# kristofbc/physical-interaction-video-prediction

Measured on AMD Instinct MI355X. Metric: predicted frames/sec (64x64x3, 10-step rollout), higher is better.
Workload: dtype f32; 1 GPU; CDNA rollout forward (Model.__call__, feed-self), batch 32/GPU, 10-frame 64x64x3 sequences, action-conditioned, num_masks=10, random-init weights; global_batch=32, parallelism=replicas x1

## Files before the change

physical-interaction-video-prediction_amd/csrc/igemm_small.hip:

```cpp
#include <stdlib.h>
#include <type_traits>

#include "pivp_kernels.h"

namespace pivp {

namespace {
constexpr int SP = 36;
constexpr int TILE = 32 * SP;
}

template <int NTB, bool IN_LN = false, bool FUSE3 = false>
__global__ __launch_bounds__(256) void igemm_small_kernel(const IgemmDesc d) {
    static_assert(!FUSE3 || NTB == 2, "the fused 1x1 needs all 64 channels of a pixel in one block");
    const int bx = blockIdx.x, by = blockIdx.y, gdy = gridDim.y;
    PIVP_SET_MAIN_PRIO();
    constexpr int BN = 32 * NTB;
    constexpr int RP = BN + 4;
    constexpr int A_OFF = 0, B_OFF = 2 * TILE;
    constexpr int STAGE_FLOATS = 2 * TILE + 2 * NTB * TILE, RED_FLOATS = 4 * 32 * RP;
    __shared__ __attribute__((aligned(16))) float lds[STAGE_FLOATS > RED_FLOATS ? STAGE_FLOATS : RED_FLOATS];
    const int tid = threadIdx.x, lane = tid & 63;
    const int wave = __builtin_amdgcn_readfirstlane(tid >> 6);
    const int half = lane >> 5, l31 = lane & 31;
    const int n_nblk = d.n_mblk;
    const int mblk = pivp_fdiv(bx, d.fd_mb_mul, d.fd_mb_sh), nblk = bx - mblk * n_nblk;
    const int m0 = mblk * 32;
    const int phase = by, py = phase >> 1, px = phase & 1;
    const bool deconv = d.deconv != 0;
    const int nty = deconv ? 1 + py : d.ksize, ntx = deconv ? 1 + px : d.ksize;
    const int ncc = (d.c0 + d.c1) >> 5;
    const int nchunks = nty * ntx * ncc;
    const int HWg = d.Hg * d.Wg;

    constexpr unsigned OOB = 0xC0000000u;
    const int cvec = tid & 7, prow = tid >> 3;
    const __amdgpu_buffer_rsrc_t rs0 = __builtin_amdgcn_make_buffer_rsrc(const_cast<float*>(d.x0), 0, d.bytes0, 0x00020000);
    const __amdgpu_buffer_rsrc_t rs1 = __builtin_amdgcn_make_buffer_rsrc(const_cast<float*>(d.c1 ? d.x1 : d.x0), 0, d.c1 ? d.bytes1 : d.bytes0, 0x00020000);
    const __amdgpu_buffer_rsrc_t rsw = __builtin_amdgcn_make_buffer_rsrc(const_cast<float*>(d.w), 0, d.bytesw, 0x00020000);
    int a_off0 = 0, a_off1 = 0, a_iy0 = -(1 << 20), a_ix0 = 0, a_pix0 = 0;
    auto anchor = [&]() {
        const int m = m0 + prow;
        if (m < d.M) {
            const int b = pivp_fdiv(m, d.fd_hw_mul, d.fd_hw_sh), rem = m - b * HWg;
            const int ay = pivp_fdiv(rem, d.fd_w_mul, d.fd_w_sh), ax = rem - ay * d.Wg;
            a_iy0 = ay * d.in_step; a_ix0 = ax * d.in_step;
            const int pix = b * d.Hin * d.Win + a_iy0 * d.Win + a_ix0;
            a_pix0 = pix;
            a_off0 = (pix * d.ld0 + cvec * 4) * 4;
            a_off1 = (pix * d.ld1 + cvec * 4) * 4;
        }
    };
    int b_goff[NTB];
#pragma unroll
    for (int t = 0; t < NTB; ++t) b_goff[t] = ((nblk * BN + t * 32 + prow) * 32 + cvec * 4) * 4;
    const int lds_w = prow * SP + cvec * 4;

    constexpr bool in_ln = IN_LN;
    __shared__ float in_stat[2];
    const __amdgpu_buffer_rsrc_t rsg = __builtin_amdgcn_make_buffer_rsrc(const_cast<float*>(in_ln ? d.in_g : d.x0), 0, in_ln ? d.Hin * d.Win * d.c0 * 4 : 0, 0x00020000);
    const __amdgpu_buffer_rsrc_t rsb = __builtin_amdgcn_make_buffer_rsrc(const_cast<float*>(in_ln ? d.in_b : d.x0), 0, in_ln ? d.Hin * d.Win * d.c0 * 4 : 0, 0x00020000);
    if (IN_LN && tid < 64) {
        float mean, rstd;
        ln_merge_partials(d.in_part, pivp_fdiv(m0, d.fd_hw_mul, d.fd_hw_sh), d.in_np, d.in_eps, mean, rstd);
        if (tid == 0) {
            in_stat[0] = mean; in_stat[1] = rstd;
            const int bs = pivp_fdiv(m0, d.fd_hw_mul, d.fd_hw_sh);
            if (d.in_stat_out && nblk == 0 && m0 == bs * HWg) { d.in_stat_out[bs * 2] = mean; d.in_stat_out[bs * 2 + 1] = rstd; }
        }
    }
    int l_cc = 0, l_ty = 0, l_tx = 0;
    constexpr int NS = 4;
    f32x4 ras[NS], rbs[NS][NTB];
    f32x4 rgs[NS], rbe[NS];
    int roo[NS];
    auto load_next = [&](auto SET, auto PART) {
        constexpr int part = decltype(PART)::value;
        f32x4& ra = ras[decltype(SET)::value];
        f32x4 (&rb)[NTB] = rbs[decltype(SET)::value];
        int dy, dx, wi;
        if (deconv) {
            const int ky = py ? 2 * l_ty : 1, kx = px ? 2 * l_tx : 1;
            dy = (py + 1 - ky) >> 1; dx = (px + 1 - kx) >> 1; wi = ky * 3 + kx;
        } else {
            dy = l_ty - d.pad; dx = l_tx - d.pad; wi = l_ty * d.ksize + l_tx;
        }
        const int ch = l_cc << 5;
        const bool first = ch < d.c0;
        const int ld = first ? d.ld0 : d.ld1;
        const int delta = ((dy * d.Win + dx) * ld + (first ? ch : ch - d.c0)) * 4;
        const int wbase = (wi * (d.wcin >> 5) + l_cc) * (d.wN ? d.wN : d.N) * 128;
        if constexpr (part != 1) {
            const int iy = a_iy0 + dy, ix = a_ix0 + dx;
            const bool ok = (unsigned)iy < (unsigned)d.Hin && (unsigned)ix < (unsigned)d.Win;
            const unsigned off = ok ? (unsigned)((first ? a_off0 : a_off1) + delta) : OOB;
            ra = __builtin_bit_cast(f32x4, first ? __builtin_amdgcn_raw_buffer_load_b128(rs0, off, 0, 0)
                                                 : __builtin_amdgcn_raw_buffer_load_b128(rs1, off, 0, 0));
            if constexpr (IN_LN) {
                const bool own = d.in_out && nblk == 0 && ok && l_ty >= 1 && l_tx >= 1 && l_ty < nty;
                roo[decltype(SET)::value] = own ? (a_pix0 + dy * d.Win + dx) * d.in_out_ld + ch + cvec * 4 : -1;
                const unsigned goff = ok ? (unsigned)(((iy * d.Win + ix) * d.c0 + ch + cvec * 4) * 4) : OOB;
                rgs[decltype(SET)::value] = __builtin_bit_cast(f32x4, __builtin_amdgcn_raw_buffer_load_b128(rsg, goff, 0, 0));
                rbe[decltype(SET)::value] = __builtin_bit_cast(f32x4, __builtin_amdgcn_raw_buffer_load_b128(rsb, goff, 0, 0));
            }
        }
        if constexpr (part != 2) {
#pragma unroll
            for (int t = 0; t < NTB; ++t) rb[t] = __builtin_bit_cast(f32x4, __builtin_amdgcn_raw_buffer_load_b128(rsw, b_goff[t], wbase, 0));
        }
        if constexpr (part != 1) { if (++l_cc == ncc) { l_cc = 0; if (++l_tx == ntx) { l_tx = 0; ++l_ty; } } }
    };
    auto store_regs = [&](auto SET, int buf) {
        f32x4 ra = ras[decltype(SET)::value];
        const f32x4 (&rb)[NTB] = rbs[decltype(SET)::value];
        if constexpr (IN_LN) {
            const float mean = in_stat[0], rstd = in_stat[1];
            const f32x4 g = rgs[decltype(SET)::value], be = rbe[decltype(SET)::value];
#pragma unroll
            for (int e = 0; e < 4; ++e) ra[e] = (ra[e] - mean) * rstd * g[e] + be[e];
            if (d.in_out && roo[decltype(SET)::value] >= 0) *reinterpret_cast<f32x4*>(d.in_out + roo[decltype(SET)::value]) = ra;
        }
        *reinterpret_cast<f32x4*>(lds + A_OFF + buf * TILE + lds_w) = ra;
#pragma unroll
        for (int t = 0; t < NTB; ++t) *reinterpret_cast<f32x4*>(lds + B_OFF + (buf * NTB + t) * TILE + lds_w) = rb[t];
    };

    if (nchunks > 0) load_next(std::integral_constant<int, 0>{}, std::integral_constant<int, 1>{});
    __builtin_amdgcn_sched_barrier(0);
    anchor();
    float f3w[FUSE3 ? 16 : 1], f3c = 0.f;
    if constexpr (FUSE3) {
        const int col = 16 * wave + (lane & 15), kg = lane >> 4, bs = pivp_fdiv(m0, d.fd_hw_mul, d.fd_hw_sh);
#pragma unroll
        for (int s4 = 0; s4 < 16; ++s4) f3w[s4] = d.f3_w[(4 * s4 + kg) * 64 + col];
        f3c = d.f3_b[col];
        if (d.f3_use_state) {
#pragma unroll
            for (int j = 0; j < 10; ++j) f3c = fmaf(j < 5 ? d.f3_action[bs * 5 + j] : d.f3_state[bs * 5 + j - 5], d.f3_w[(64 + j) * 64 + col], f3c);
        }
    }
    f32x16 acc[NTB];
#pragma unroll
    for (int t = 0; t < NTB; ++t)
#pragma unroll
        for (int r = 0; r < 16; ++r) acc[t][r] = 0.f;
    const int frag = l31 * SP + 8 * wave + 4 * half;

    if (nchunks > 0) {
        using S0 = std::integral_constant<int, 0>; using S1 = std::integral_constant<int, 1>;
        using P0 = std::integral_constant<int, 0>; using P2 = std::integral_constant<int, 2>;
        auto mma = [&](int buf) {
            const f32x4 fa = *reinterpret_cast<const f32x4*>(lds + A_OFF + buf * TILE + frag);
            f32x4 fb[NTB];
#pragma unroll
            for (int t = 0; t < NTB; ++t) fb[t] = *reinterpret_cast<const f32x4*>(lds + B_OFF + (buf * NTB + t) * TILE + frag);
#pragma unroll
            for (int s2 = 0; s2 < 4; ++s2)
#pragma unroll
                for (int t = 0; t < NTB; ++t) acc[t] = __builtin_amdgcn_mfma_f32_32x32x2f32(fa[s2], fb[t][s2], acc[t], 0, 0, 0);
        };
        using S2 = std::integral_constant<int, 2>; using S3 = std::integral_constant<int, 3>;
        load_next(S0{}, P2{});
        load_next(S1{}, P0{});
        load_next(S2{}, P0{});
        load_next(S3{}, P0{});
        if constexpr (IN_LN) __syncthreads();
        store_regs(S0{}, 0);
        __syncthreads();
        auto trip = [&](auto SET, auto NEXT) {
            constexpr int buf = decltype(SET)::value & 1;
            load_next(SET, P0{});
            mma(buf);
            store_regs(NEXT, buf ^ 1);
            __syncthreads();
        };
        int it = 0;
        for (; it + NS <= nchunks; it += NS) { trip(S0{}, S1{}); trip(S1{}, S2{}); trip(S2{}, S3{}); trip(S3{}, S0{}); }
        if (it < nchunks) trip(S0{}, S1{});
        if (it + 1 < nchunks) trip(S1{}, S2{});
        if (it + 2 < nchunks) trip(S2{}, S3{});
    }

#pragma unroll
    for (int t = 0; t < NTB; ++t)
#pragma unroll
        for (int r = 0; r < 16; ++r) {
            const int m = (r & 3) + 8 * (r >> 2) + 4 * half;
            lds[(wave * 32 + m) * RP + t * 32 + l31] = acc[t][r];
        }
    __syncthreads();
    const int m = m0 + prow;
    const bool valid = m < d.M;
    const int b = valid ? pivp_fdiv(m, d.fd_hw_mul, d.fd_hw_sh) : 0, rem = m - b * HWg;
    const int ay = pivp_fdiv(rem, d.fd_w_mul, d.fd_w_sh), ax = rem - ay * d.Wg;
    const int oy0 = deconv ? py : 0, ox0 = deconv ? px : 0;
    float* orow = d.out + ((size_t)(b * d.Hout + ay * d.out_step + oy0) * d.Wout + ax * d.out_step + ox0) * d.ldo + nblk * BN;
    float sv[4 * NTB];
#pragma unroll
    for (int t = 0; t < NTB; ++t) {
        const int cl = t * 32 + cvec * 4;
        f32x4 v = *reinterpret_cast<const f32x4*>(lds + prow * RP + cl);
#pragma unroll
        for (int w = 1; w < 4; ++w) v += *reinterpret_cast<const f32x4*>(lds + (w * 32 + prow) * RP + cl);
        if (d.bias) v += *reinterpret_cast<const f32x4*>(d.bias + nblk * BN + cl);
        if (d.relu) { v[0] = fmaxf(v[0], 0.f); v[1] = fmaxf(v[1], 0.f); v[2] = fmaxf(v[2], 0.f); v[3] = fmaxf(v[3], 0.f); }
        if (valid) {
            if (d.accum) v += *reinterpret_cast<const f32x4*>(orow + cl);
            *reinterpret_cast<f32x4*>(orow + cl) = v;
        }
#pragma unroll
        for (int e = 0; e < 4; ++e) sv[t * 4 + e] = v[e];
    }
    if constexpr (FUSE3) {
        __syncthreads();
#pragma unroll
        for (int t = 0; t < NTB; ++t)
            *reinterpret_cast<f32x4*>(lds + prow * 68 + t * 32 + cvec * 4) = f32x4{sv[t * 4], sv[t * 4 + 1], sv[t * 4 + 2], sv[t * 4 + 3]};
        __syncthreads();
        const int li = lane & 15, kg = lane >> 4;
        f32x4 c3[2];
        c3[0] = f32x4{f3c, f3c, f3c, f3c}; c3[1] = c3[0];
#pragma unroll
        for (int s4 = 0; s4 < 16; ++s4) {
#pragma unroll
            for (int mt = 0; mt < 2; ++mt)
                c3[mt] = __builtin_amdgcn_mfma_f32_16x16x4f32(lds[(16 * mt + li) * 68 + 4 * s4 + kg], f3w[s4], c3[mt], 0, 0, 0);
        }
#pragma unroll
        for (int mt = 0; mt < 2; ++mt)
#pragma unroll
            for (int r = 0; r < 4; ++r) {
                const int mm = m0 + 16 * mt + 4 * kg + r;
                if (mm < d.M) d.f3_out[(size_t)mm * 64 + 16 * wave + li] = fmaxf(c3[mt][r], 0.f);
            }
        const int bs3 = pivp_fdiv(m0, d.fd_hw_mul, d.fd_hw_sh);
        if (d.f3_state_out && m0 == bs3 * HWg && tid < 5) {
            const int bs = bs3;
            float v = d.f3_bcs[tid];
#pragma unroll
            for (int j = 0; j < 10; ++j) v = fmaf(d.f3_wcs[tid * 10 + j], j < 5 ? d.f3_action[bs * 5 + j] : d.f3_state[bs * 5 + j - 5], v);
            d.f3_state_out[bs * 5 + tid] = v;
        }
    }
    if (d.ln_part) {
        __syncthreads();
        float s1 = 0.f;
#pragma unroll
        for (int i = 0; i < 4 * NTB; ++i) s1 += valid ? sv[i] : 0.f;
        s1 = wave_sum(s1);
        const float c1 = wave_sum(valid ? (float)(4 * NTB) : 0.f);
        if (lane == 0) { lds[wave] = s1; lds[4 + wave] = c1; }
        __syncthreads();
        const float cnt = (lds[4] + lds[5]) + (lds[6] + lds[7]);
        const float mean = ((lds[0] + lds[1]) + (lds[2] + lds[3])) / cnt;
        float q = 0.f;
#pragma unroll
        for (int i = 0; i < 4 * NTB; ++i) { const float dd = sv[i] - mean; q = valid ? fmaf(dd, dd, q) : q; }
        q = wave_sum(q);
        if (lane == 0) lds[8 + wave] = q;
        __syncthreads();
        if (tid == 0) {
            const int bb = pivp_fdiv(m0, d.fd_hw_mul, d.fd_hw_sh);
            float* pp = d.ln_part + ((size_t)bb * d.ln_nparts + (((m0 - bb * HWg) >> 5) * n_nblk + nblk) * gdy + phase) * 4;
            pp[0] = cnt; pp[1] = mean; pp[2] = (lds[8] + lds[9]) + (lds[10] + lds[11]); pp[3] = 0.f;
        }
    }
}

int igemm_small(const IgemmDesc& d, hipStream_t stream, int* ln_nparts) {
    PIVP_CHECK_ARG(d.ldo % 4 == 0 && ((uintptr_t)d.out & 15) == 0 && (!d.bias || ((uintptr_t)d.bias & 15) == 0));
    const int mblk = (d.M + 31) / 32, nt = d.N / 32;
    int ntb = small_ntb(d.M, nt, d.nphase);
    if (d.f3_out) {
        PIVP_CHECK_ARG(d.in_g && nt == 2 && d.nphase == 1 && (d.Hg * d.Wg) % 32 == 0 && !d.accum && !d.ln_part);
        PIVP_CHECK_ARG(d.f3_w && d.f3_b && d.f3_action && d.f3_state && (!d.f3_state_out || (d.f3_wcs && d.f3_bcs)));
        ntb = 2;
    }
    dim3 grid(mblk * (nt / ntb), d.nphase);
    IgemmDesc dd = d;
    const int hwg = d.Hg * d.Wg;
    const int np = (hwg / 32) * (nt / ntb) * d.nphase;
    dd.ln_nparts = (d.ln_part && hwg % 32 == 0 && np <= d.ln_cap) ? np : 0;
    if (!dd.ln_nparts) dd.ln_part = nullptr;
    if (ln_nparts) *ln_nparts = dd.ln_nparts;
    dd.n_mblk = nt / ntb;
    pivp_fastdiv((unsigned)(nt / ntb), &dd.fd_mb_mul, &dd.fd_mb_sh);
    pivp_fastdiv((unsigned)hwg, &dd.fd_hw_mul, &dd.fd_hw_sh);
    pivp_fastdiv((unsigned)d.Wg, &dd.fd_w_mul, &dd.fd_w_sh);
    if (d.in_g) {
        PIVP_CHECK_ARG(igemm_in_ln_ok(d) && d.in_b && d.in_part && d.in_np > 0);
        PIVP_CHECK_ARG(!d.in_out || (d.ksize == 3 && d.pad == 1 && d.in_step == 2 && d.Hin == 2 * d.Hg && d.Win == 2 * d.Wg && d.in_out_ld >= d.c0 && d.in_out_ld % 4 == 0 &&
                                     ((uintptr_t)d.in_out & 15) == 0 && (long long)d.B * d.Hin * d.Win * d.in_out_ld < (1LL << 31)));
        if (d.f3_out) { hipLaunchKernelGGL((igemm_small_kernel<2, true, true>), grid, dim3(256), 0, stream, dd); return PIVP_LAUNCH_STATUS(); }
        if (ntb == 3) hipLaunchKernelGGL((igemm_small_kernel<3, true>), grid, dim3(256), 0, stream, dd);
        else if (ntb == 2) hipLaunchKernelGGL((igemm_small_kernel<2, true>), grid, dim3(256), 0, stream, dd);
        else hipLaunchKernelGGL((igemm_small_kernel<1, true>), grid, dim3(256), 0, stream, dd);
        return PIVP_LAUNCH_STATUS();
    }
    if (ntb == 3) hipLaunchKernelGGL(igemm_small_kernel<3>, grid, dim3(256), 0, stream, dd);
    else if (ntb == 2) hipLaunchKernelGGL(igemm_small_kernel<2>, grid, dim3(256), 0, stream, dd);
    else hipLaunchKernelGGL(igemm_small_kernel<1>, grid, dim3(256), 0, stream, dd);
    return PIVP_LAUNCH_STATUS();
}

bool igemm_in_ln_ok(const IgemmDesc& d) {
    return !d.deconv && d.nphase == 1 && d.c1 == 0 && d.ld0 == d.c0 && (d.Hg * d.Wg) % 32 == 0 && d.M == d.B * d.Hg * d.Wg &&
           (long long)d.Hin * d.Win * d.c0 * 4 < (1LL << 31);
}

}

PIVP_DEFINE_MAIN_PRIO_SETTER(igemm_small)
```

Before: 35300 frames/s.

## Run fused 1x1 igemm variant with eight waves splitting output columns

For the FUSE3 (conv plus fused 1x1) kernel, the block grows from 256 to 512 threads. The waves split into four K-groups by two column tiles, so each wave holds one accumulator instead of two. The waves for column 1 load the weight tiles while column-0 waves load and LayerNorm the activations, and the fused 1x1 MFMA epilogue is split across the column tiles. This raises parallelism and latency hiding in a small-grid kernel, at the cost of more threads per block, specialised load roles and dropping the in_out path for this variant.

```diff
diff --git a/physical-interaction-video-prediction_amd/csrc/igemm_small.hip b/physical-interaction-video-prediction_amd/csrc/igemm_small.hip
--- a/physical-interaction-video-prediction_amd/csrc/igemm_small.hip
+++ b/physical-interaction-video-prediction_amd/csrc/igemm_small.hip
@@ -11,8 +11,10 @@
 }
 
 template <int NTB, bool IN_LN = false, bool FUSE3 = false>
-__global__ __launch_bounds__(256) void igemm_small_kernel(const IgemmDesc d) {
-    static_assert(!FUSE3 || NTB == 2, "the fused 1x1 needs all 64 channels of a pixel in one block");
+__global__ __launch_bounds__(FUSE3 ? 512 : 256) void igemm_small_kernel(const IgemmDesc d) {
+    static_assert(!FUSE3 || (NTB == 2 && IN_LN), "the fused 1x1 needs all 64 channels of a pixel in one block, and has the LayerNorm-on-load form only");
+    constexpr bool W8 = FUSE3;
+    constexpr int NTW = W8 ? 1 : NTB;
     const int bx = blockIdx.x, by = blockIdx.y, gdy = gridDim.y;
     PIVP_SET_MAIN_PRIO();
     constexpr int BN = 32 * NTB;
@@ -22,6 +24,8 @@
     __shared__ __attribute__((aligned(16))) float lds[STAGE_FLOATS > RED_FLOATS ? STAGE_FLOATS : RED_FLOATS];
     const int tid = threadIdx.x, lane = tid & 63;
     const int wave = __builtin_amdgcn_readfirstlane(tid >> 6);
+    const int kgrp = W8 ? wave & 3 : wave;
+    const int wcol = W8 ? wave >> 2 : 0;
     const int half = lane >> 5, l31 = lane & 31;
     const int n_nblk = d.n_mblk;
     const int mblk = pivp_fdiv(bx, d.fd_mb_mul, d.fd_mb_sh), nblk = bx - mblk * n_nblk;
@@ -34,7 +38,7 @@
     const int HWg = d.Hg * d.Wg;
 
     constexpr unsigned OOB = 0xC0000000u;
-    const int cvec = tid & 7, prow = tid >> 3;
+    const int cvec = tid & 7, prow = W8 ? (tid & 255) >> 3 : tid >> 3;
     const __amdgpu_buffer_rsrc_t rs0 = __builtin_amdgcn_make_buffer_rsrc(const_cast<float*>(d.x0), 0, d.bytes0, 0x00020000);
     const __amdgpu_buffer_rsrc_t rs1 = __builtin_amdgcn_make_buffer_rsrc(const_cast<float*>(d.c1 ? d.x1 : d.x0), 0, d.c1 ? d.bytes1 : d.bytes0, 0x00020000);
     const __amdgpu_buffer_rsrc_t rsw = __builtin_amdgcn_make_buffer_rsrc(const_cast<float*>(d.w), 0, d.bytesw, 0x00020000);
@@ -60,15 +64,23 @@
     __shared__ float in_stat[2];
     const __amdgpu_buffer_rsrc_t rsg = __builtin_amdgcn_make_buffer_rsrc(const_cast<float*>(in_ln ? d.in_g : d.x0), 0, in_ln ? d.Hin * d.Win * d.c0 * 4 : 0, 0x00020000);
     const __amdgpu_buffer_rsrc_t rsb = __builtin_amdgcn_make_buffer_rsrc(const_cast<float*>(in_ln ? d.in_b : d.x0), 0, in_ln ? d.Hin * d.Win * d.c0 * 4 : 0, 0x00020000);
-    if (IN_LN && tid < 64) {
-        float mean, rstd;
-        ln_merge_partials(d.in_part, pivp_fdiv(m0, d.fd_hw_mul, d.fd_hw_sh), d.in_np, d.in_eps, mean, rstd);
-        if (tid == 0) {
-            in_stat[0] = mean; in_stat[1] = rstd;
-            const int bs = pivp_fdiv(m0, d.fd_hw_mul, d.fd_hw_sh);
-            if (d.in_stat_out && nblk == 0 && m0 == bs * HWg) { d.in_stat_out[bs * 2] = mean; d.in_stat_out[bs * 2 + 1] = rstd; }
-        }
-    }
+    auto merge_stats = [&]() {
+        if (IN_LN && tid < 64) {
+            float mean, rstd;
+            ln_merge_partials(d.in_part, pivp_fdiv(m0, d.fd_hw_mul, d.fd_hw_sh), d.in_np, d.in_eps, mean, rstd);
+            if (tid == 0) {
+                in_stat[0] = mean; in_stat[1] = rstd;
+                const int bs = pivp_fdiv(m0, d.fd_hw_mul, d.fd_hw_sh);
+                if (d.in_stat_out && nblk == 0 && m0 == bs * HWg) { d.in_stat_out[bs * 2] = mean; d.in_stat_out[bs * 2 + 1] = rstd; }
+            }
+        }
+    };
+    if constexpr (!W8) merge_stats();
+    const bool wts = W8 && wcol != 0;
+    const int ln_bytes = W8 ? d.Hin * d.Win * d.c0 * 4 : 0;
+    const __amdgpu_buffer_rsrc_t rq0 = __builtin_amdgcn_make_buffer_rsrc(const_cast<float*>(wts ? d.w : d.x0), 0, wts ? d.bytesw : d.bytes0, 0x00020000);
+    const __amdgpu_buffer_rsrc_t rq1 = __builtin_amdgcn_make_buffer_rsrc(const_cast<float*>(wts ? d.w : W8 ? d.in_g : d.x0), 0, wts ? d.bytesw : ln_bytes, 0x00020000);
+    const __amdgpu_buffer_rsrc_t rq2 = __builtin_amdgcn_make_buffer_rsrc(const_cast<float*>(W8 ? d.in_b : d.x0), 0, wts ? 0 : ln_bytes, 0x00020000);
     int l_cc = 0, l_ty = 0, l_tx = 0;
     constexpr int NS = 4;
     f32x4 ras[NS], rbs[NS][NTB];
@@ -90,6 +102,19 @@
         const int ld = first ? d.ld0 : d.ld1;
         const int delta = ((dy * d.Win + dx) * ld + (first ? ch : ch - d.c0)) * 4;
         const int wbase = (wi * (d.wcin >> 5) + l_cc) * (d.wN ? d.wN : d.N) * 128;
+        if constexpr (W8) {
+            static_assert(part == 0, "the eight-wave form requests whole chunks");
+            const int iy = a_iy0 + dy, ix = a_ix0 + dx;
+            const bool ok = (unsigned)iy < (unsigned)d.Hin && (unsigned)ix < (unsigned)d.Win;
+            const unsigned aoff = ok ? (unsigned)(a_off0 + delta) : OOB;
+            const unsigned goff = ok ? (unsigned)(((iy * d.Win + ix) * d.c0 + ch + cvec * 4) * 4) : OOB;
+            const int so = wcol ? wbase : 0;
+            ra = __builtin_bit_cast(f32x4, __builtin_amdgcn_raw_buffer_load_b128(rq0, wcol ? (unsigned)b_goff[0] : aoff, so, 0));
+            rgs[decltype(SET)::value] = __builtin_bit_cast(f32x4, __builtin_amdgcn_raw_buffer_load_b128(rq1, wcol ? (unsigned)b_goff[1] : goff, so, 0));
+            rbe[decltype(SET)::value] = __builtin_bit_cast(f32x4, __builtin_amdgcn_raw_buffer_load_b128(rq2, wcol ? OOB : goff, 0, 0));
+            if (++l_cc == ncc) { l_cc = 0; if (++l_tx == ntx) { l_tx = 0; ++l_ty; } }
+            return;
+        }
         if constexpr (part != 1) {
             const int iy = a_iy0 + dy, ix = a_ix0 + dx;
             const bool ok = (unsigned)iy < (unsigned)d.Hin && (unsigned)ix < (unsigned)d.Win;
@@ -113,6 +138,19 @@
     auto store_regs = [&](auto SET, int buf) {
         f32x4 ra = ras[decltype(SET)::value];
         const f32x4 (&rb)[NTB] = rbs[decltype(SET)::value];
+        if constexpr (W8) {
+            const f32x4 g = rgs[decltype(SET)::value], be = rbe[decltype(SET)::value];
+            if (wcol) {
+                *reinterpret_cast<f32x4*>(lds + B_OFF + (buf * NTB + 0) * TILE + lds_w) = ra;
+                *reinterpret_cast<f32x4*>(lds + B_OFF + (buf * NTB + 1) * TILE + lds_w) = g;
+            } else {
+                const float mean = in_stat[0], rstd = in_stat[1];
+#pragma unroll
+                for (int e = 0; e < 4; ++e) ra[e] = (ra[e] - mean) * rstd * g[e] + be[e];
+                *reinterpret_cast<f32x4*>(lds + A_OFF + buf * TILE + lds_w) = ra;
+            }
+            return;
+        }
         if constexpr (IN_LN) {
             const float mean = in_stat[0], rstd = in_stat[1];
             const f32x4 g = rgs[decltype(SET)::value], be = rbe[decltype(SET)::value];
@@ -125,12 +163,22 @@
         for (int t = 0; t < NTB; ++t) *reinterpret_cast<f32x4*>(lds + B_OFF + (buf * NTB + t) * TILE + lds_w) = rb[t];
     };
 
-    if (nchunks > 0) load_next(std::integral_constant<int, 0>{}, std::integral_constant<int, 1>{});
+    if constexpr (!W8) {
+        if (nchunks > 0) load_next(std::integral_constant<int, 0>{}, std::integral_constant<int, 1>{});
+    }
     __builtin_amdgcn_sched_barrier(0);
     anchor();
+    if constexpr (W8) {
+        if (nchunks > 0) {
+            load_next(std::integral_constant<int, 0>{}, std::integral_constant<int, 0>{});
+            load_next(std::integral_constant<int, 1>{}, std::integral_constant<int, 0>{});
+            load_next(std::integral_constant<int, 2>{}, std::integral_constant<int, 0>{});
+            load_next(std::integral_constant<int, 3>{}, std::integral_constant<int, 0>{});
+        }
+    }
     float f3w[FUSE3 ? 16 : 1], f3c = 0.f;
     if constexpr (FUSE3) {
-        const int col = 16 * wave + (lane & 15), kg = lane >> 4, bs = pivp_fdiv(m0, d.fd_hw_mul, d.fd_hw_sh);
+        const int col = 16 * kgrp + (lane & 15), kg = lane >> 4, bs = pivp_fdiv(m0, d.fd_hw_mul, d.fd_hw_sh);
 #pragma unroll
         for (int s4 = 0; s4 < 16; ++s4) f3w[s4] = d.f3_w[(4 * s4 + kg) * 64 + col];
         f3c = d.f3_b[col];
@@ -139,31 +187,35 @@
             for (int j = 0; j < 10; ++j) f3c = fmaf(j < 5 ? d.f3_action[bs * 5 + j] : d.f3_state[bs * 5 + j - 5], d.f3_w[(64 + j) * 64 + col], f3c);
         }
     }
-    f32x16 acc[NTB];
-#pragma unroll
-    for (int t = 0; t < NTB; ++t)
+    f32x16 acc[NTW];
+#pragma unroll
+    for (int t = 0; t < NTW; ++t)
 #pragma unroll
         for (int r = 0; r < 16; ++r) acc[t][r] = 0.f;
-    const int frag = l31 * SP + 8 * wave + 4 * half;
+    const int frag = l31 * SP + 8 * kgrp + 4 * half;
 
     if (nchunks > 0) {
         using S0 = std::integral_constant<int, 0>; using S1 = std::integral_constant<int, 1>;
         using P0 = std::integral_constant<int, 0>; using P2 = std::integral_constant<int, 2>;
         auto mma = [&](int buf) {
             const f32x4 fa = *reinterpret_cast<const f32x4*>(lds + A_OFF + buf * TILE + frag);
-            f32x4 fb[NTB];
-#pragma unroll
-            for (int t = 0; t < NTB; ++t) fb[t] = *reinterpret_cast<const f32x4*>(lds + B_OFF + (buf * NTB + t) * TILE + frag);
+            f32x4 fb[NTW];
+#pragma unroll
+            for (int t = 0; t < NTW; ++t) fb[t] = *reinterpret_cast<const f32x4*>(lds + B_OFF + (buf * NTB + (W8 ? wcol : t)) * TILE + frag);
 #pragma unroll
             for (int s2 = 0; s2 < 4; ++s2)
 #pragma unroll
-                for (int t = 0; t < NTB; ++t) acc[t] = __builtin_amdgcn_mfma_f32_32x32x2f32(fa[s2], fb[t][s2], acc[t], 0, 0, 0);
+                for (int t = 0; t < NTW; ++t) acc[t] = __builtin_amdgcn_mfma_f32_32x32x2f32(fa[s2], fb[t][s2], acc[t], 0, 0, 0);
         };
         using S2 = std::integral_constant<int, 2>; using S3 = std::integral_constant<int, 3>;
-        load_next(S0{}, P2{});
-        load_next(S1{}, P0{});
-        load_next(S2{}, P0{});
-        load_next(S3{}, P0{});
+        if constexpr (!W8) {
+            load_next(S0{}, P2{});
+            load_next(S1{}, P0{});
+            load_next(S2{}, P0{});
+            load_next(S3{}, P0{});
+        } else {
+            merge_stats();
+        }
         if constexpr (IN_LN) __syncthreads();
         store_regs(S0{}, 0);
         __syncthreads();
@@ -182,11 +234,11 @@
     }
 
 #pragma unroll
-    for (int t = 0; t < NTB; ++t)
+    for (int t = 0; t < NTW; ++t)
 #pragma unroll
         for (int r = 0; r < 16; ++r) {
             const int m = (r & 3) + 8 * (r >> 2) + 4 * half;
-            lds[(wave * 32 + m) * RP + t * 32 + l31] = acc[t][r];
+            lds[(kgrp * 32 + m) * RP + (W8 ? wcol : t) * 32 + l31] = acc[t][r];
         }
     __syncthreads();
     const int m = m0 + prow;
@@ -195,10 +247,10 @@
     const int ay = pivp_fdiv(rem, d.fd_w_mul, d.fd_w_sh), ax = rem - ay * d.Wg;
     const int oy0 = deconv ? py : 0, ox0 = deconv ? px : 0;
     float* orow = d.out + ((size_t)(b * d.Hout + ay * d.out_step + oy0) * d.Wout + ax * d.out_step + ox0) * d.ldo + nblk * BN;
-    float sv[4 * NTB];
-#pragma unroll
-    for (int t = 0; t < NTB; ++t) {
-        const int cl = t * 32 + cvec * 4;
+    float sv[4 * NTW];
+#pragma unroll
+    for (int t = 0; t < NTW; ++t) {
+        const int cl = (W8 ? wcol : t) * 32 + cvec * 4;
         f32x4 v = *reinterpret_cast<const f32x4*>(lds + prow * RP + cl);
 #pragma unroll
         for (int w = 1; w < 4; ++w) v += *reinterpret_cast<const f32x4*>(lds + (w * 32 + prow) * RP + cl);
@@ -213,26 +265,18 @@
     }
     if constexpr (FUSE3) {
         __syncthreads();
-#pragma unroll
-        for (int t = 0; t < NTB; ++t)
-            *reinterpret_cast<f32x4*>(lds + prow * 68 + t * 32 + cvec * 4) = f32x4{sv[t * 4], sv[t * 4 + 1], sv[t * 4 + 2], sv[t * 4 + 3]};
-        __syncthreads();
-        const int li = lane & 15, kg = lane >> 4;
-        f32x4 c3[2];
-        c3[0] = f32x4{f3c, f3c, f3c, f3c}; c3[1] = c3[0];
-#pragma unroll
-        for (int s4 = 0; s4 < 16; ++s4) {
-#pragma unroll
-            for (int mt = 0; mt < 2; ++mt)
-                c3[mt] = __builtin_amdgcn_mfma_f32_16x16x4f32(lds[(16 * mt + li) * 68 + 4 * s4 + kg], f3w[s4], c3[mt], 0, 0, 0);
-        }
-#pragma unroll
-        for (int mt = 0; mt < 2; ++mt)
-#pragma unroll
-            for (int r = 0; r < 4; ++r) {
-                const int mm = m0 + 16 * mt + 4 * kg + r;
-                if (mm < d.M) d.f3_out[(size_t)mm * 64 + 16 * wave + li] = fmaxf(c3[mt][r], 0.f);
-            }
+        *reinterpret_cast<f32x4*>(lds + prow * 68 + wcol * 32 + cvec * 4) = f32x4{sv[0], sv[1], sv[2], sv[3]};
+        __syncthreads();
+        const int li = lane & 15, kg = lane >> 4, mt = wcol;
+        f32x4 c3 = f32x4{f3c, f3c, f3c, f3c};
+#pragma unroll
+        for (int s4 = 0; s4 < 16; ++s4)
+            c3 = __builtin_amdgcn_mfma_f32_16x16x4f32(lds[(16 * mt + li) * 68 + 4 * s4 + kg], f3w[s4], c3, 0, 0, 0);
+#pragma unroll
+        for (int r = 0; r < 4; ++r) {
+            const int mm = m0 + 16 * mt + 4 * kg + r;
+            if (mm < d.M) d.f3_out[(size_t)mm * 64 + 16 * kgrp + li] = fmaxf(c3[r], 0.f);
+        }
         const int bs3 = pivp_fdiv(m0, d.fd_hw_mul, d.fd_hw_sh);
         if (d.f3_state_out && m0 == bs3 * HWg && tid < 5) {
             const int bs = bs3;
@@ -242,20 +286,20 @@
             d.f3_state_out[bs * 5 + tid] = v;
         }
     }
-    if (d.ln_part) {
+    if (!W8 && d.ln_part) {
         __syncthreads();
         float s1 = 0.f;
 #pragma unroll
-        for (int i = 0; i < 4 * NTB; ++i) s1 += valid ? sv[i] : 0.f;
+        for (int i = 0; i < 4 * NTW; ++i) s1 += valid ? sv[i] : 0.f;
         s1 = wave_sum(s1);
-        const float c1 = wave_sum(valid ? (float)(4 * NTB) : 0.f);
+        const float c1 = wave_sum(valid ? (float)(4 * NTW) : 0.f);
         if (lane == 0) { lds[wave] = s1; lds[4 + wave] = c1; }
         __syncthreads();
         const float cnt = (lds[4] + lds[5]) + (lds[6] + lds[7]);
         const float mean = ((lds[0] + lds[1]) + (lds[2] + lds[3])) / cnt;
         float q = 0.f;
 #pragma unroll
-        for (int i = 0; i < 4 * NTB; ++i) { const float dd = sv[i] - mean; q = valid ? fmaf(dd, dd, q) : q; }
+        for (int i = 0; i < 4 * NTW; ++i) { const float dd = sv[i] - mean; q = valid ? fmaf(dd, dd, q) : q; }
         q = wave_sum(q);
         if (lane == 0) lds[8 + wave] = q;
         __syncthreads();
@@ -272,7 +316,7 @@
     const int mblk = (d.M + 31) / 32, nt = d.N / 32;
     int ntb = small_ntb(d.M, nt, d.nphase);
     if (d.f3_out) {
-        PIVP_CHECK_ARG(d.in_g && nt == 2 && d.nphase == 1 && (d.Hg * d.Wg) % 32 == 0 && !d.accum && !d.ln_part);
+        PIVP_CHECK_ARG(d.in_g && nt == 2 && d.nphase == 1 && (d.Hg * d.Wg) % 32 == 0 && !d.accum && !d.ln_part && !d.in_out);
         PIVP_CHECK_ARG(d.f3_w && d.f3_b && d.f3_action && d.f3_state && (!d.f3_state_out || (d.f3_wcs && d.f3_bcs)));
         ntb = 2;
     }
@@ -291,7 +335,7 @@
         PIVP_CHECK_ARG(igemm_in_ln_ok(d) && d.in_b && d.in_part && d.in_np > 0);
         PIVP_CHECK_ARG(!d.in_out || (d.ksize == 3 && d.pad == 1 && d.in_step == 2 && d.Hin == 2 * d.Hg && d.Win == 2 * d.Wg && d.in_out_ld >= d.c0 && d.in_out_ld % 4 == 0 &&
                                      ((uintptr_t)d.in_out & 15) == 0 && (long long)d.B * d.Hin * d.Win * d.in_out_ld < (1LL << 31)));
-        if (d.f3_out) { hipLaunchKernelGGL((igemm_small_kernel<2, true, true>), grid, dim3(256), 0, stream, dd); return PIVP_LAUNCH_STATUS(); }
+        if (d.f3_out) { hipLaunchKernelGGL((igemm_small_kernel<2, true, true>), grid, dim3(512), 0, stream, dd); return PIVP_LAUNCH_STATUS(); }
         if (ntb == 3) hipLaunchKernelGGL((igemm_small_kernel<3, true>), grid, dim3(256), 0, stream, dd);
         else if (ntb == 2) hipLaunchKernelGGL((igemm_small_kernel<2, true>), grid, dim3(256), 0, stream, dd);
         else hipLaunchKernelGGL((igemm_small_kernel<1, true>), grid, dim3(256), 0, stream, dd);
```

Result: no change. 35310 frames/s, median of 2 (+0.0%).
